# SutirthaChakraborty/RTFS-Net

Hardware: AMD Instinct MI355X
Metric: mixtures/sec forward (2 s@16 kHz, 2-spk) RTFS-Net-4 (higher is better)
Workload: dtype f32 (f16x3 split-precision MFMA products, f32 accumulate; every tensor in HBM is f32)

## Files before the change

### include/rtfs_amd.h

```cpp
#ifndef RTFS_AMD_H
#define RTFS_AMD_H
#include <stddef.h>
#ifdef __cplusplus
extern "C" {
#endif

enum rtfs_pack_kind {
    RTFS_PACK_ENCODER = 0,
    RTFS_PACK_AUDIO_BN = 1,
    RTFS_PACK_BLOCK = 2,
    RTFS_PACK_DUALPATH = 3,
    RTFS_PACK_ATTENTION = 4,
    RTFS_PACK_TFAR = 5,
    RTFS_PACK_CAF = 6,
    RTFS_PACK_S3 = 7,
    RTFS_PACK_DECODER = 8,
    RTFS_PACK_BLOCK_LSTM = 9,
    RTFS_PACK_DUALPATH_LSTM = 10
};

const char* rtfs_version(void);
size_t rtfs_pack_floats(int kind);
int rtfs_num_frames(int L);

// ... 20 lines not shown
int rtfs_tf_attention_f32(const float* x, const float* pack, float* out, int B, int T, void* ws, size_t ws_bytes,
                          void* stream);

size_t rtfs_tfar_workspace_bytes(int B, int H, int W, int Hg, int Wg);
int rtfs_tfar_f32(const float* local, const float* global, const float* pack, float* out, int B, int H, int W, int Hg,
                  int Wg, void* ws, size_t ws_bytes, void* stream);

size_t rtfs_caf_workspace_bytes(int B, int Tv);
int rtfs_caf_f32(const float* audio, const float* video, const float* pack, float* out, int B, int T, int F, int Tv,
                 void* ws, size_t ws_bytes, void* stream);

size_t rtfs_vp_pack_floats(void);
int rtfs_vp_block_f32(const float* video, const float* pack, float* out, int B, int Tv, void* stream);

int rtfs_s3_mask_f32(const float* refined, const float* a0, const float* pack, float* out, int B, int T, int F,
                     void* stream);

size_t rtfs_istft_decoder_workspace_bytes(int B, int T);
int rtfs_istft_decoder_f32(const float* x, const float* pack, float* wav, int B, int T, int L, void* ws, size_t ws_bytes,
                           void* stream);

size_t rtfs_separator_workspace_bytes(int B, int L, int Tv);
int rtfs_set_batch_split(int n);
size_t rtfs_separator_workspace_bytes_ex(int B, int L, int Tv, int split);
int rtfs_separator_forward_ex_f32(const float* wav, const float* video_vp, const float* pack_enc, const float* pack_bn,
                                  const float* pack_block, const float* pack_caf, const float* pack_s3,
                                  const float* pack_dec, float* out, int B, int L, int Tv, int repeats, void* ws,
                                  size_t ws_bytes, void* stream, void* video_ready, int rnn_kind, int split);
int rtfs_separator_forward_f32(const float* wav, const float* video_vp, const float* pack_enc, const float* pack_bn,
                               const float* pack_block, const float* pack_caf, const float* pack_s3,
                               const float* pack_dec, float* out, int B, int L, int Tv, int repeats, void* ws,
                               size_t ws_bytes, void* stream, void* video_ready, int rnn_kind );

size_t rtfs_separator_speakers_workspace_bytes(int B, int K, int L, int Tv, int split);
int rtfs_separator_speakers_f32(const float* wav, const float* video_vp, const float* pack_enc, const float* pack_bn,
                                const float* pack_block, const float* pack_caf, const float* pack_s3, const float* pack_dec,
                                float* out, int B, int K, int L, int Tv, int repeats, void* ws, size_t ws_bytes, void* stream,
                                void* video_ready, int rnn_kind, int split);

size_t rtfs_separator_targets_workspace_bytes(const int* counts, int B, int L, int Tv, int split);
int rtfs_separator_targets_f32(const float* wav, const float* video_vp, const int* counts, const int* mix_of, const float* pack_enc,
                               const float* pack_bn, const float* pack_block, const float* pack_caf, const float* pack_s3,
                               const float* pack_dec, float* out, int B, int N, int L, int Tv, int repeats, void* ws, size_t ws_bytes,
                               void* stream, void* video_ready, int rnn_kind, int split);

size_t rtfs_sru_workspace_bytes(int L, int N);
// ... 269 lines not shown
```

### rtfs-net_amd/_lib.py

```python
from __future__ import annotations

import ctypes as C
import os
import threading

import torch

_HERE = os.path.dirname(os.path.abspath(__file__))
LIB_PATH = os.path.join(_HERE, "librtfs_amd.so")

PACK_ENCODER, PACK_AUDIO_BN, PACK_BLOCK, PACK_DUALPATH, PACK_ATTENTION, PACK_TFAR, PACK_CAF, PACK_S3, PACK_DECODER, PACK_BLOCK_LSTM, PACK_DUALPATH_LSTM = range(11)

_ERR = {-1: "bad shape", -2: "workspace too small", -3: "kernel launch failure", -4: "bad argument"}

_p, _i, _z = C.c_void_p, C.c_int, C.c_size_t
SIGNATURES = {
    "rtfs_version": (C.c_char_p, []),
    "rtfs_pack_floats": (_z, [_i]),
    "rtfs_num_frames": (_i, [_i]),
    "rtfs_stft_encoder_workspace_bytes": (_z, [_i, _i]),
    "rtfs_stft_encoder_f32": (_i, [_p, _p, _p, _p, _i, _i, _p, _z, _p]),
    "rtfs_audio_bottleneck_workspace_bytes": (_z, [_i]),
    "rtfs_audio_bottleneck_f32": (_i, [_p, _p, _p, _p, _i, _i, _i, _p, _z, _p]),
    "rtfs_block_workspace_bytes": (_z, [_i, _i, _i]),
    "rtfs_block_f32": (_i, [_p, _p, _p, _p, _i, _i, _i, _p, _z, _p, _i]),
    "rtfs_dualpath_workspace_bytes": (_z, [_i, _i, _i]),
    "rtfs_dualpath_sru_f32": (_i, [_p, _p, _p, _i, _i, _i, _i, _p, _z, _p]),
    "rtfs_dualpath_lstm_f32": (_i, [_p, _p, _p, _i, _i, _i, _i, _p, _z, _p]),
    "rtfs_tf_attention_workspace_bytes": (_z, [_i, _i]),
    "rtfs_tf_attention_f32": (_i, [_p, _p, _p, _i, _i, _p, _z, _p]),
    "rtfs_tfar_workspace_bytes": (_z, [_i, _i, _i, _i, _i]),
    "rtfs_tfar_f32": (_i, [_p, _p, _p, _p, _i, _i, _i, _i, _i, _p, _z, _p]),
    "rtfs_caf_workspace_bytes": (_z, [_i, _i]),
    "rtfs_caf_f32": (_i, [_p, _p, _p, _p, _i, _i, _i, _i, _p, _z, _p]),
    "rtfs_vp_pack_floats": (_z, []),
    "rtfs_vp_block_f32": (_i, [_p, _p, _p, _i, _i, _p]),
    "rtfs_s3_mask_f32": (_i, [_p, _p, _p, _p, _i, _i, _i, _p]),
    "rtfs_istft_decoder_workspace_bytes": (_z, [_i, _i]),
    "rtfs_istft_decoder_f32": (_i, [_p, _p, _p, _i, _i, _i, _p, _z, _p]),
    "rtfs_separator_workspace_bytes": (_z, [_i, _i, _i]),
    "rtfs_set_batch_split": (_i, [_i]),
    "rtfs_debug_launch_count": (C.c_ulonglong, []),
    "rtfs_separator_workspace_bytes_ex": (_z, [_i, _i, _i, _i]),
    "rtfs_separator_forward_ex_f32": (_i, [_p] * 9 + [_i, _i, _i, _i, _p, _z, _p, _p, _i, _i]),
    "rtfs_separator_forward_f32": (_i, [_p] * 9 + [_i, _i, _i, _i, _p, _z, _p, _p, _i]),
    "rtfs_separator_speakers_workspace_bytes": (_z, [_i, _i, _i, _i, _i]),
    "rtfs_separator_speakers_f32": (_i, [_p] * 9 + [_i, _i, _i, _i, _i, _p, _z, _p, _p, _i, _i]),
    "rtfs_separator_targets_workspace_bytes": (_z, [_p, _i, _i, _i, _i]),
    "rtfs_separator_targets_f32": (_i, [_p] * 11 + [_i, _i, _i, _i, _i, _p, _z, _p, _p, _i, _i]),
    "rtfs_sru_workspace_bytes": (_z, [_i, _i]),
    "rtfs_sru_f32": (_i, [_p, _p, _p, _i, _i, _p, _z, _p]),
    "rtfs_sru_train_pack_floats": (_z, []),
    "rtfs_sru_grad_floats": (_z, []),
    "rtfs_sru_saved_floats": (_z, [_i, _i]),
    "rtfs_sru_backward_workspace_bytes": (_z, [_i, _i]),
    "rtfs_sru_forward_train_f32": (_i, [_p, _p, _p, _p, _i, _i, _p]),
    "rtfs_sru_backward_f32": (_i, [_p, _p, _p, _p, _p, _p, _i, _i, _p, _z, _p]),
    **{f"rtfs_dualpath_{infix}{name}": sig for infix in ("", "lstm_", "gru_") for name, sig in (
        ("train_pack_floats", (_z, [])),
        ("grad_floats", (_z, [])),
        ("saved_floats", (_z, [_i, _i, _i, _i])),
        ("train_workspace_bytes", (_z, [_i, _i, _i, _i])),
        ("forward_train_f32", (_i, [_p, _p, _p, _p, _i, _i, _i, _i, _p, _z, _p])),
        ("backward_f32", (_i, [_p, _p, _p, _p, _p, _p, _i, _i, _i, _i, _p, _z, _p])))},
# ... 232 lines not shown
```

### rtfs-net_amd/csrc/api.hip

```cpp
#include "api_common.h"
#include <atomic>
#include <vector>

namespace {

struct Cursor {
    const float* p;
    size_t off = 0;
    explicit Cursor(const float* base) : p(base) {}
    const float* take(size_t n) {
        const float* r = p ? p + off : nullptr;
        off += (n + 63) / 64 * 64;
        return r;
    }
};

struct Fork {
    hipStream_t st = nullptr;
    RtfsSide side{};
    bool open = false;
    int begin(hipStream_t owner, int slot) {
        st = owner;
        CHECK(rtfs_side_stream(owner, slot, &side));
        if (hipEventRecord(side.fork, st) != hipSuccess || hipStreamWaitEvent(side.stream, side.fork, 0) != hipSuccess) return RTFS_ERR_LAUNCH;
// ... 309 lines not shown
        a.wt = p.proj_wt;
        a.w16 = p.proj_w16;
        a.bias = p.proj_b;
        a.out = w.x_enc;
        a.gw = p.gw;
        a.gb = p.gb;
        a.slope = p.gslope;
        a.P = P;
        a.cs = w.cs;
        a.tile_ctr = ctr;
        if (caf && !gemm_f32()) {
            a.caf_r = caf->r_out; a.caf_att = caf->att_out;
            a.caf_w_key = caf->w_key; a.caf_bn_key = caf->bn_key; a.caf_w_val = caf->w_val; a.caf_bn_val = caf->bn_val;
            a.caf_T = caf->T; a.caf_F = caf->F; a.caf_Tv = caf->Tv;
        }
        if (gemm_f32()) return launch_pw_gateway_proj(a, B, st);
        const int rc = launch_pws_head4(a, B, st);
        if (rc == RTFS_ERR_ARG) CHECK(launch_pws_gateway_proj(a, B, st));
        else CHECK(rc);
    }
    return RTFS_OK;
}

int block_body(const BlockPack& p, int B, int T, int F, const BlockWs& w, hipStream_t st, bool zero_stats = true) {
    const int Tp = T / 2, Fp = F / 2;
    const int P = T * F, Pg = Tp * Fp;
    const double icF = 1.0 / ((double)CH * P), icG = 1.0 / ((double)CH * Pg);
    typedef BlockWs W;
    constexpr int TH_A = 24, TH_B = 24, TH_C = 12, TH_G = 64, TH_S = 64;
    if (zero_stats && hipMemsetAsync(w.stats, 0, sizeof(double) * W::NSTAT * w.Bfull * 2, st) != hipSuccess) return RTFS_ERR_LAUNCH;
    {
        DwArgs a;
        a.x = w.x_enc;
        a.w[0] = p.ds0_w;
        a.bias[0] = p.ds0_b;
        a.out[0] = w.c0;
        a.stats_out[0] = w.st(W::S_C0, B);
        a.C = CH; a.H = T; a.W = F; a.TH = TH_A; a.cs = w.cs;
        CHECK(launch_dw_s1(a, 1, false, 0, B, st));
    }
    DwArgs s14;
    s14.x = w.c0;
    s14.in_stats = w.st(W::S_C0, B); s14.in_inv_count = icF; s14.in_gamma = p.ds0_g; s14.in_beta = p.ds0_be;
    s14.C = CH; s14.H = T; s14.W = F; s14.TH = 64; s14.Hg = Tp; s14.Wg = Fp; s14.cs = w.cs;
    s14.w[0] = p.fus0.loc_w;
    s14.stats_out[0] = w.st(W::S_L0, B);
    s14.rev = 1;
    DwArgs s3;
    s3.x = w.c0;
    s3.in_stats = w.st(W::S_C0, B); s3.in_inv_count = icF; s3.in_gamma = p.ds0_g; s3.in_beta = p.ds0_be;
    s3.w[0] = p.ds1_w;
    s3.bias[0] = p.ds1_b;
// ... 68 lines not shown
        a.w[0] = p.cat0.emb_w; a.w[1] = p.cat0.gate_w;
        a.out[0] = w.E2; a.out[1] = w.G2;
        a.stats_out[0] = w.st(W::S_E2, B); a.stats_out[1] = w.st(W::S_G2, B);
        a.C = CH; a.H = Tp; a.W = Fp; a.TH = TH_G;
        if (Fp >= 16) {
            CHECK(launch_dw_s1(a, 2, false, 0, B, st));
        } else {
            GCombineArgs g;
            g.l = w.L1; g.gate = w.G1; g.emb = w.E1;
            g.l_stats = a.loc_stats; g.gate_stats = a.gate_stats; g.emb_stats = a.emb_stats;
            g.l_gamma = a.loc_gamma; g.l_beta = a.loc_beta; g.gate_gamma = a.gate_gamma; g.gate_beta = a.gate_beta; g.emb_gamma = a.emb_gamma; g.emb_beta = a.emb_beta;
            g.inv_count = icG;
            g.out = w.xf1;
            g.C = CH; g.HW = Pg;
            CHECK(launch_g_combine(g, B, st));
            a.x = w.xf1; a.gate = nullptr; a.emb = nullptr; a.in_combine = 0;
            CHECK(launch_dw_s1(a, 2, false, 0, B, st));
        }
    }
    DwArgs d0in;
    d0in.x = w.c0;
    d0in.in_stats = w.st(W::S_C0, B); d0in.in_inv_count = icF; d0in.in_gamma = p.ds0_g; d0in.in_beta = p.ds0_be;
    d0in.C = CH; d0in.H = T; d0in.W = F; d0in.TH = 64; d0in.Hg = Tp; d0in.Wg = Fp; d0in.cs = w.cs;
    {
        DwArgs a = d0in;
        a.w[0] = p.fus0.loc_w;
        a.loc_stats = w.st(W::S_L0, B); a.loc_inv_count = icF; a.loc_gamma = p.fus0.loc_g; a.loc_beta = p.fus0.loc_b;
        a.gate = w.G0; a.gate_stats = w.st(W::S_G0, B); a.gate_gamma = p.fus0.gate_g; a.gate_beta = p.fus0.gate_b;
        a.emb = w.E0; a.emb_stats = w.st(W::S_E0, B); a.emb_gamma = p.fus0.emb_g; a.emb_beta = p.fus0.emb_b;
        a.g_inv_count = icG;
        a.out[0] = w.xf0;
        a.TH = TH_B;
        CHECK(launch_dw_s1(a, 1, true, 2, B, st));
    }
    DwArgs xin;
    xin.x = w.xf0;
    xin.C = CH; xin.H = T; xin.W = F; xin.TH = 64; xin.Hg = Tp; xin.Wg = Fp; xin.cs = w.cs;
    {
        DwArgs a = xin;
        a.w[0] = p.cat0.loc_w;
        a.stats_out[0] = w.st(W::S_L2, B);
        a.rev = 1;
        a.TH = TH_S;
        CHECK(launch_dw_s1(a, 1, false, 1, B, st));
    }
    {
        DwArgs a = xin;
        a.w[0] = p.cat0.loc_w;
        a.loc_stats = w.st(W::S_L2, B); a.loc_inv_count = icF; a.loc_gamma = p.cat0.loc_g; a.loc_beta = p.cat0.loc_b;
        a.gate = w.G2; a.gate_stats = w.st(W::S_G2, B); a.gate_gamma = p.cat0.gate_g; a.gate_beta = p.cat0.gate_b;
        a.emb = w.E2; a.emb_stats = w.st(W::S_E2, B); a.emb_gamma = p.cat0.emb_g; a.emb_beta = p.cat0.emb_b;
        a.g_inv_count = icG;
        a.addend = w.c0; a.add_stats = w.st(W::S_C0, B); a.add_inv_count = icF; a.add_gamma = p.ds0_g; a.add_beta = p.ds0_be;
        a.out[0] = w.expanded;
        a.rev = 1;
        a.TH = TH_B;
        CHECK(launch_dw_s1(a, 1, false, 2, B, st));
    }
    return RTFS_OK;
}

int block_tail(const BlockPack& p, float* out, int B, int T, int F, BlockWs& w, hipStream_t st, unsigned* ctr = nullptr) {
    const int P = T * F;
    {
        PwArgs a;
        a.x = w.expanded;
        a.wt = p.res_wt;
        a.w16 = p.res_w16;
        a.bias = p.res_b;
        a.aux = w.residual;
        a.out = out;
        a.P = P;
        a.cs = w.cs;
        a.tile_ctr = ctr;
        CHECK(gemm_f32() ? launch_pw_residual(a, B, st) : launch_pws_residual(a, B, st));
    }
    return RTFS_OK;
}

int block_forward(const BlockPack& p, const float* x, const float* x_res, float* out, int B, int T, int F, BlockWs& w, hipStream_t st,
                  const CafArgs* caf = nullptr) {
// ... 481 lines not shown
                CHECK(block_tail(pk, cur, B, T, NF, w.blk, st, f.tile_ctr));
            }
        }
    }
    if (!gemm_f32()) {
        PwArgs a;
        a.x = cur; a.bias = ps.bias; a.aux = w.a0; a.out = w.z; a.slope = ps.slope; a.P = P; a.cs = cs; a.w16 = ps.w16; a.w16b = pd.w16p; a.cout_live = 18;
        a.tile_ctr = nctr < 64 ? w.ctr + nctr++ : nullptr;
        a.stats = w.st0; a.inv_count = 1.0 / ((double)CA * P);
        CHECK(launch_pwr_s3_taps(a, B, st));
        return launch_dec_istft(w.z, out, B, T, NF, L, (size_t)cs, (size_t)18 * cs, st);
    }
    CHECK(s3_mask(ps, cur, w.a0, nxt, B, P, st));
    return decoder(pd, nxt, out, w.z, B, T, L, st);
}
}

static std::atomic<int> g_split{0};
int rtfs_set_batch_split(int n) {
    if (n < 0 || n > 8) return RTFS_ERR_ARG;
    g_split.store(n);
    return RTFS_OK;
}
static int separator_parts(int B, int split = 0) {
    static const int env = getenv("RTFS_SPLIT") ? atoi(getenv("RTFS_SPLIT")) : 0;
    int n = split > 0 ? split : g_split.load();
    if (n <= 0) n = env > 0 ? env : 1;
    while (n > 1 && B / n < 8) --n;
    return n;
}

size_t rtfs_separator_workspace_bytes(int B, int L, int Tv) { return rtfs_separator_workspace_bytes_ex(B, L, Tv, 0); }

size_t rtfs_separator_workspace_bytes_ex(int B, int L, int Tv, int split) {
    if (split < 0 || split > 8) return 0;
    Arena ar(nullptr, 0);
    const int T = rtfs_num_frames(L), np = separator_parts(B, split);
    for (int i = 0; i < np; ++i) SepWs w(ar, (B * (i + 1)) / np - (B * i) / np, T, Tv, pitch(T * NF));
    return ar.off + 256;
}

int rtfs_separator_forward_f32(const float* wav, const float* video_vp, const float* pack_enc, const float* pack_bn, const float* pack_block,
                               const float* pack_caf, const float* pack_s3, const float* pack_dec, float* out, int B, int L, int Tv,
                               int repeats, void* ws, size_t ws_bytes, void* stream, void* video_ready, int rnn_kind) {
    return rtfs_separator_forward_ex_f32(wav, video_vp, pack_enc, pack_bn, pack_block, pack_caf, pack_s3, pack_dec, out, B, L, Tv, repeats, ws, ws_bytes,
                                         stream, video_ready, rnn_kind, 0);
// ... 150 lines not shown
    a.in_stats = (const double*)p[1]; a.in_gamma = (const float*)p[2]; a.in_beta = (const float*)p[3];
    for (int k = 0; k < 4; ++k) {
        a.w[k] = (const float*)p[4 + k];
        a.bias[k] = (present >> k) & 1 ? (const float*)p[8 + k] : nullptr;
        a.out[k] = (float*)p[12 + k];
        a.stats_out[k] = (double*)p[16 + k];
    }
    a.loc_stats = (const double*)p[20]; a.loc_gamma = (const float*)p[21]; a.loc_beta = (const float*)p[22];
    a.gate = (const float*)p[23]; a.gate_stats = (const double*)p[24]; a.gate_gamma = (const float*)p[25]; a.gate_beta = (const float*)p[26];
    a.emb = (const float*)p[27]; a.emb_stats = (const double*)p[28]; a.emb_gamma = (const float*)p[29]; a.emb_beta = (const float*)p[30];
    if ((present >> 4) & 1) {
        a.addend = (const float*)p[31]; a.add_stats = (const double*)p[32]; a.add_gamma = (const float*)p[33]; a.add_beta = (const float*)p[34];
    }
    a.C = n[1]; a.H = n[2]; a.W = n[3]; a.Hg = n[4]; a.Wg = n[5]; a.TH = n[6]; a.cs = n[7]; a.rev = n[8]; a.in_combine = n[12];
    a.in_inv_count = d[0]; a.loc_inv_count = d[1]; a.g_inv_count = d[2]; a.add_inv_count = d[3];
    return a;
}
}

int rtfs_debug_dw_f32(int op, void* const* ptrs, int n_ptrs, const int* ints, int n_ints, const double* dbls, int n_dbls, int* route,
                      int route_cap, void* stream) {
    RTFS_RETURN_IF(!ptrs || !ints || !dbls || !route || route_cap < 1 + 8 * 4, RTFS_ERR_ARG);
    route[0] = 0;
    const int jobs = op == 1 || op == 2 ? 2 : 1;
    int rc;
    if (op >= 0 && op <= 3) {
        RTFS_RETURN_IF(n_ptrs < jobs * DW_DBG_PTRS || n_ints < jobs * DW_DBG_INTS || n_dbls < jobs * DW_DBG_DBLS, RTFS_ERR_ARG);
        const int B = ints[0];
        RTFS_RETURN_IF(B < 1 || ints[1] < 1 || ints[2] < 1 || ints[3] < 1, RTFS_ERR_ARG);
        const DwArgs a = dw_debug_args(ptrs, ints, dbls);
        if (op == 0) {
            rc = launch_dw_s1(a, ints[9], ints[10] != 0, ints[11], B, S(stream));
        } else if (op == 3) {
            rc = launch_dw_s2_pool(a, B, S(stream));
        } else {
            const DwArgs b = dw_debug_args(ptrs + DW_DBG_PTRS, ints + DW_DBG_INTS, dbls + DW_DBG_DBLS);
            rc = op == 1 ? launch_dw_g3(a, b, B, S(stream)) : launch_dw_s2_stats(a, b, B, S(stream));
        }
    } else if (op == 4) {
        RTFS_RETURN_IF(n_ptrs < 6 || n_ints < 3 || n_dbls < 1 || ints[0] < 1 || ints[1] < 1 || ints[2] < 1, RTFS_ERR_ARG);
        rc = launch_g_form((const float*)ptrs[0], (const float*)ptrs[1], (const double*)ptrs[2], dbls[0], (const float*)ptrs[3],
                           (const float*)ptrs[4], (float*)ptrs[5], ints[0], ints[1], ints[2], S(stream));
    } else if (op == 5) {
        RTFS_RETURN_IF(n_ptrs < 13 || n_ints < 3 || n_dbls < 1 || ints[0] < 1 || ints[1] < 1 || ints[2] < 1, RTFS_ERR_ARG);
        GCombineArgs g;
        g.l = (const float*)ptrs[0]; g.gate = (const float*)ptrs[1]; g.emb = (const float*)ptrs[2];
        g.l_stats = (const double*)ptrs[3]; g.gate_stats = (const double*)ptrs[4]; g.emb_stats = (const double*)ptrs[5];
        g.l_gamma = (const float*)ptrs[6]; g.l_beta = (const float*)ptrs[7]; g.gate_gamma = (const float*)ptrs[8];
        g.gate_beta = (const float*)ptrs[9]; g.emb_gamma = (const float*)ptrs[10]; g.emb_beta = (const float*)ptrs[11];
        g.out = (float*)ptrs[12];
        g.inv_count = dbls[0];
        g.C = ints[1]; g.HW = ints[2];
        rc = launch_g_combine(g, ints[0], S(stream));
    } else {
        return RTFS_ERR_ARG;
    }
    const DwRoute& r = dw_route_last();
    route[0] = r.n;
    for (int i = 0; i < r.n; ++i) {
        const DwRouteJob& j = r.job[i];
        const int v[8] = {j.family, j.nconv, j.in_affine, j.mode, j.var, j.TH, j.gx, j.gy};
// ... 230 lines not shown
```

### rtfs-net_amd/csrc/k_dw.hip

```cpp
#include "common.h"
#include "kernels.h"

template <int NCONV, bool IN_AFFINE, int MODE>
__device__ __forceinline__ void dw_s1_body(const DwArgs& a, const float* __restrict__ X, const float* __restrict__ GATE,
                                           const float* __restrict__ EMB, const float* __restrict__ ADD, float* __restrict__ O0,
                                           float* __restrict__ O1, float* __restrict__ O2, float* __restrict__ O3) {
    __shared__ double red[8];
    const int H = a.H, W = a.W, C = a.C;
    const int b = blockIdx.z;
    const int g = blockIdx.x * 256 + threadIdx.x;
    const bool live = g < C * W;
    const int c = live ? g / W : 0, f = live ? g - c * W : 0;
    const int r0 = blockIdx.y * a.TH, r1 = min(r0 + a.TH, H);
    const size_t plane = ((size_t)b * C + c) * (size_t)a.cs;
    const float* __restrict__ xp = X + plane;
    float isc = 1.f, ish = 0.f;
    if (IN_AFFINE) gln_fold(a.in_stats + 2 * b, a.in_inv_count, a.in_gamma[c], a.in_beta[c], isc, ish);
    float wgt[NCONV][16], bia[NCONV];
#pragma unroll
    for (int n = 0; n < NCONV; ++n) {
#pragma unroll
        for (int j = 0; j < 16; ++j) wgt[n][j] = a.w[n][c * 16 + j];
        bia[n] = a.bias[n] ? a.bias[n][c] : 0.f;
    }
// ... 452 lines not shown
    if (MODE != 2) {
#pragma unroll
        for (int n = 0; n < NCONV; ++n) {
            block_stats_atomic(s2[n].x + s2[n].y, ss2[n].x + ss2[n].y, red, a.stats_out[n] + 2 * b);
            __syncthreads();
        }
    }
}

template <int NCONV, bool IN_AFFINE, int MODE, int VAR = 0>
__global__ __launch_bounds__(256, NCONV == 1 && MODE != 2 ? 4 : 2) void dw1p_kernel(DwArgs a) {
    dw1p_body<NCONV, IN_AFFINE, MODE, VAR>(a, a.x, a.gate, a.emb, a.addend, a.out[0], a.out[1], a.out[2], a.out[3]);
}

template <int V>
__global__ __launch_bounds__(256, 2) void dw_g3_kernel(DwArgs a0, DwArgs a1, DwArgs a2) {
    int id = blockIdx.x;
    if (DW_XCD) id = (id & 7) * (int)(gridDim.x >> 3) + (id >> 3);
    if (id < a1.blk0) dw1p_body<2, false, 0, V>(a0, a0.x, a0.gate, a0.emb, a0.addend, a0.out[0], a0.out[1], a0.out[2], a0.out[3]);
    else if (id < a2.blk0) dw1p_body<2, false, 0, V>(a1, a1.x, a1.gate, a1.emb, a1.addend, a1.out[0], a1.out[1], a1.out[2], a1.out[3]);
    else dw1p_body<1, true, 0, V>(a2, a2.x, a2.gate, a2.emb, a2.addend, a2.out[0], a2.out[1], a2.out[2], a2.out[3]);
}

__device__ __forceinline__ void dw_s2_pool_body(const DwArgs& a, const float* __restrict__ X, float* __restrict__ O0, float* __restrict__ O1) {
    __shared__ double red[8];
    const int H = a.H, W = a.W, C = a.C, Ho = a.Hg, Wo = a.Wg;
    const int b = blockIdx.z;
    const int g = blockIdx.x * 256 + threadIdx.x;
    const bool live = g < C * Wo;
    const int c = live ? g / Wo : 0, j = live ? g - c * Wo : 0;
    const int i0 = blockIdx.y * a.TH, i1 = min(i0 + a.TH, Ho);
    const size_t plane = ((size_t)b * C + c) * (size_t)a.cs;
    const float* __restrict__ xp = X + plane;
    float isc, ish;
    gln_fold(a.in_stats + 2 * b, a.in_inv_count, a.in_gamma[c], a.in_beta[c], isc, ish);
    float wgt[16];
#pragma unroll
    for (int k = 0; k < 16; ++k) wgt[k] = a.w[0][c * 16 + k];
    const float bia = a.bias[0][c];
    const int fs = (int)(((long long)j * W) / Wo), fe = (int)(((long long)(j + 1) * W + Wo - 1) / Wo);
    bool fok[4], fpool[4];
    int fcl[4];
#pragma unroll
    for (int d = 0; d < 4; ++d) {
        const int f = 2 * j - 1 + d;
        fok[d] = live && f >= 0 && f < W;
// ... 403 lines not shown
            if (nconv == 2) return a.in_combine ? launch_dw1p_t<2, false, 0, 4>(a, B, st) : launch_dw1p_t<2, false, 0>(a, B, st);
            if (nconv == 4) {
                DwArgs b = a;
                for (int i = 0; i < 2; ++i) {
                    b.w[i] = a.w[2 + i]; b.bias[i] = a.bias[2 + i]; b.out[i] = a.out[2 + i]; b.stats_out[i] = a.stats_out[2 + i];
                }
                const int rc = launch_dw1p_t<2, false, 0>(a, B, st);
                return rc ? rc : launch_dw1p_t<2, false, 0>(b, B, st);
            }
        }
    }
    if (mode == 0 && nconv == 1 && !in_affine) return launch_dw_s1_t<1, false, 0>(a, B, st);
    if (mode == 0 && nconv == 1 && in_affine) return launch_dw_s1_t<1, true, 0>(a, B, st);
    if (mode == 0 && nconv == 2 && !in_affine) return launch_dw_s1_t<2, false, 0>(a, B, st);
    if (mode == 0 && nconv == 4 && !in_affine) return launch_dw_s1_t<4, false, 0>(a, B, st);
    if (mode == 0 && nconv == 3 && !in_affine) return launch_dw_s1_t<3, false, 0>(a, B, st);
    if (mode == 1 && nconv == 1 && in_affine) return launch_dw_s1_t<1, true, 1>(a, B, st);
    if (mode == 1 && nconv == 1 && !in_affine) return launch_dw_s1_t<1, false, 1>(a, B, st);
    if (mode == 2 && nconv == 1 && in_affine) return launch_dw_s1_t<1, true, 2>(a, B, st);
    if (mode == 2 && nconv == 1 && !in_affine) return launch_dw_s1_t<1, false, 2>(a, B, st);
    return RTFS_ERR_ARG;
}

int launch_dw_g3(const DwArgs& conv4, const DwArgs& aff1, int B, hipStream_t st) {
    route_clear();
    DwArgs j[3] = {conv4, conv4, aff1};
    const bool nohalo = 64 % ((conv4.W + 1) / 2) == 0 && conv4.W == aff1.W;
    for (int i = 0; i < 2; ++i) {
        j[1].w[i] = conv4.w[2 + i]; j[1].bias[i] = conv4.bias[2 + i]; j[1].out[i] = conv4.out[2 + i]; j[1].stats_out[i] = conv4.stats_out[2 + i];
    }
    int off = 0;
    for (int i = 0; i < 3; ++i) {
        DwArgs& a = j[i];
        if (a.W < 16 || (a.cs && a.cs < a.H * a.W)) return RTFS_ERR_ARG;
        if (!a.cs) a.cs = a.H * a.W;
        if ((size_t)a.C * a.cs * 4 >= ((size_t)1 << 31)) return RTFS_ERR_ARG;
        a.rev = 0;
        a.gx = cdiv(cdiv(a.C * ((a.W + 1) / 2), nohalo ? 64 : DW1P_PAIRS), 4);
        a.TH = band_rows(a.TH, a.H, a.gx, 3 * B, 640);
        a.gy = cdiv(a.H, a.TH);
        a.nblk = a.gx * a.gy * B;
        a.blk0 = off;
        off += a.nblk;
    }
    for (int i = 0; i < 3; ++i) route_add(DW_FAM_G3, i < 2 ? 2 : 1, i == 2, 0, nohalo ? 16 : 0, j[i].TH, j[i].gx, j[i].gy);
    if (nohalo) hipLaunchKernelGGL(dw_g3_kernel<16>, dim3((off + 7) / 8 * 8), dim3(256), 0, st, j[0], j[1], j[2]);
// ... 130 lines not shown
```

### rtfs-net_amd/csrc/kernels.h

```cpp
#pragma once
#include <hip/hip_runtime.h>
#include <stddef.h>
#include "common.h"

struct PwArgs {
    const float* x = nullptr;
    const float* x2 = nullptr;
    float* res_out = nullptr;
    const float* wt = nullptr;
    const void* w16 = nullptr;
    const void* w16b = nullptr;
    const float* bias = nullptr;
    const float* aux = nullptr;
    float* out = nullptr;
    const double* stats = nullptr;
    double inv_count = 0;
    const float* gamma = nullptr;
    const float* beta = nullptr;
    const float* gw = nullptr;
    const float* gb = nullptr;
    const float* slope = nullptr;
    int P = 0;
    int cs = 0;
    int cout_live = 0;
// ... 134 lines not shown
    const float* gate_beta = nullptr;
    const float* emb = nullptr;
    const double* emb_stats = nullptr;
    const float* emb_gamma = nullptr;
    const float* emb_beta = nullptr;
    double g_inv_count = 0;
    const float* addend = nullptr;
    const double* add_stats = nullptr;
    double add_inv_count = 0;
    const float* add_gamma = nullptr;
    const float* add_beta = nullptr;
};

struct GCombineArgs {
    const float *l, *gate, *emb;
    const double *l_stats, *gate_stats, *emb_stats;
    const float *l_gamma, *l_beta, *gate_gamma, *gate_beta, *emb_gamma, *emb_beta;
    double inv_count;
    float* out;
    int C, HW;
};

enum DwFamily { DW_FAM_S1 = 1, DW_FAM_1P = 2, DW_FAM_G3 = 3, DW_FAM_S2X = 4, DW_FAM_S2_POOL = 5, DW_FAM_S2_STATS = 6, DW_FAM_G_FORM = 7,
                DW_FAM_G_COMBINE = 8 };
struct DwRouteJob { int family, nconv, in_affine, mode, var, TH, gx, gy; };
struct DwRoute { int n; DwRouteJob job[4]; };
const DwRoute& dw_route_last();

int launch_dw_s1(const DwArgs& a, int nconv, bool in_affine, int mode, int B, hipStream_t st);
int launch_dw_g3(const DwArgs& conv4, const DwArgs& aff1, int B, hipStream_t st);
int launch_dw_s2_pool(const DwArgs& a, int B, hipStream_t st);
int launch_dw_s2_stats(const DwArgs& s2, const DwArgs& stats, int B, hipStream_t st);
int launch_g_form(const float* p0, const float* c1, const double* st1, double inv_count, const float* gamma,
                  const float* beta, float* g, int B, int C, int HW, hipStream_t st);
int launch_g_combine(const GCombineArgs& a, int B, hipStream_t st);
int launch_transpose(const float* x, float* y, int N, int H, int W, hipStream_t st);
int launch_stats(const float* x, double* stats, int B, size_t N, hipStream_t st);
int launch_stats2(const float* x, double* stats, int B, size_t N, double* part, hipStream_t st);

struct DpArgs {
    const float* x = nullptr;
    float* out = nullptr;
    int R = 0, Ls = 0;
    size_t bstride = 0, rstride = 0, cstride = 0;
    const float* ln_gamma = nullptr;
    const float* ln_beta = nullptr;
    const float* W0 = nullptr;
    const float* Wl = nullptr;
    const float* wc = nullptr;
    const float* bias = nullptr;
    const float* Wt = nullptr;
    const float* bt = nullptr;
    const float* whh = nullptr;
};
size_t dualpath_lds_bytes(int Ls);
// ... 308 lines not shown
```

Baseline: 3338.

## Fuse fusion, concat-stats and concat-output depthwise stages into a two-pass recompute kernel

Adds a two-pass depthwise kernel for the W=129 case that recomputes the gated fusion output xf0 on the fly in a per-wave LDS ring, instead of writing xf0 to HBM and reading it back twice. Pass 0 computes only the concat-branch statistics; pass 1 recomputes xf0, applies the second conv, gate, embedding and residual, then stages output rows through an LDS ring for coalesced stores. It is enabled when the activation footprint exceeds 256 MB, or when forced through a new API setter. Otherwise the original three launches remain. The trade-off is extra arithmetic from recomputing xf0 twice, against saving its HBM traffic at large batch.

```diff
diff --git a/include/rtfs_amd.h b/include/rtfs_amd.h
--- a/include/rtfs_amd.h
+++ b/include/rtfs_amd.h
@@ -66,6 +66,7 @@
 
 size_t rtfs_separator_workspace_bytes(int B, int L, int Tv);
 int rtfs_set_batch_split(int n);
+int rtfs_set_dw_two_pass(int mode);
 size_t rtfs_separator_workspace_bytes_ex(int B, int L, int Tv, int split);
 int rtfs_separator_forward_ex_f32(const float* wav, const float* video_vp, const float* pack_enc, const float* pack_bn,
                                   const float* pack_block, const float* pack_caf, const float* pack_s3,
diff --git a/rtfs-net_amd/_lib.py b/rtfs-net_amd/_lib.py
--- a/rtfs-net_amd/_lib.py
+++ b/rtfs-net_amd/_lib.py
@@ -40,6 +40,7 @@
     "rtfs_istft_decoder_f32": (_i, [_p, _p, _p, _i, _i, _i, _p, _z, _p]),
     "rtfs_separator_workspace_bytes": (_z, [_i, _i, _i]),
     "rtfs_set_batch_split": (_i, [_i]),
+    "rtfs_set_dw_two_pass": (_i, [_i]),
     "rtfs_debug_launch_count": (C.c_ulonglong, []),
     "rtfs_separator_workspace_bytes_ex": (_z, [_i, _i, _i, _i]),
     "rtfs_separator_forward_ex_f32": (_i, [_p] * 9 + [_i, _i, _i, _i, _p, _z, _p, _p, _i, _i]),
diff --git a/rtfs-net_amd/csrc/api.hip b/rtfs-net_amd/csrc/api.hip
--- a/rtfs-net_amd/csrc/api.hip
+++ b/rtfs-net_amd/csrc/api.hip
@@ -355,12 +355,21 @@
     return RTFS_OK;
 }
 
+static std::atomic<int> g_dw_two_pass{0};
+#ifndef RTFS_DW2P_TH_A
+#define RTFS_DW2P_TH_A 64
+#endif
+#ifndef RTFS_DW2P_TH_B
+#define RTFS_DW2P_TH_B 64
+#endif
+constexpr size_t DW_TWO_PASS_BYTES = 256u * 1000u * 1000u;
 int block_body(const BlockPack& p, int B, int T, int F, const BlockWs& w, hipStream_t st, bool zero_stats = true) {
     const int Tp = T / 2, Fp = F / 2;
     const int P = T * F, Pg = Tp * Fp;
     const double icF = 1.0 / ((double)CH * P), icG = 1.0 / ((double)CH * Pg);
     typedef BlockWs W;
     constexpr int TH_A = 24, TH_B = 24, TH_C = 12, TH_G = 64, TH_S = 64;
+    constexpr int TH_2A = RTFS_DW2P_TH_A, TH_2B = RTFS_DW2P_TH_B;
     if (zero_stats && hipMemsetAsync(w.stats, 0, sizeof(double) * W::NSTAT * w.Bfull * 2, st) != hipSuccess) return RTFS_ERR_LAUNCH;
     {
         DwArgs a;
@@ -475,41 +484,48 @@
     d0in.x = w.c0;
     d0in.in_stats = w.st(W::S_C0, B); d0in.in_inv_count = icF; d0in.in_gamma = p.ds0_g; d0in.in_beta = p.ds0_be;
     d0in.C = CH; d0in.H = T; d0in.W = F; d0in.TH = 64; d0in.Hg = Tp; d0in.Wg = Fp; d0in.cs = w.cs;
-    {
-        DwArgs a = d0in;
-        a.w[0] = p.fus0.loc_w;
-        a.loc_stats = w.st(W::S_L0, B); a.loc_inv_count = icF; a.loc_gamma = p.fus0.loc_g; a.loc_beta = p.fus0.loc_b;
-        a.gate = w.G0; a.gate_stats = w.st(W::S_G0, B); a.gate_gamma = p.fus0.gate_g; a.gate_beta = p.fus0.gate_b;
-        a.emb = w.E0; a.emb_stats = w.st(W::S_E0, B); a.emb_gamma = p.fus0.emb_g; a.emb_beta = p.fus0.emb_b;
-        a.g_inv_count = icG;
-        a.out[0] = w.xf0;
-        a.TH = TH_B;
-        CHECK(launch_dw_s1(a, 1, true, 2, B, st));
-    }
+    DwArgs f0 = d0in;
+    f0.w[0] = p.fus0.loc_w;
+    f0.loc_stats = w.st(W::S_L0, B); f0.loc_inv_count = icF; f0.loc_gamma = p.fus0.loc_g; f0.loc_beta = p.fus0.loc_b;
+    f0.gate = w.G0; f0.gate_stats = w.st(W::S_G0, B); f0.gate_gamma = p.fus0.gate_g; f0.gate_beta = p.fus0.gate_b;
+    f0.emb = w.E0; f0.emb_stats = w.st(W::S_E0, B); f0.emb_gamma = p.fus0.emb_g; f0.emb_beta = p.fus0.emb_b;
+    f0.g_inv_count = icG;
     DwArgs xin;
     xin.x = w.xf0;
     xin.C = CH; xin.H = T; xin.W = F; xin.TH = 64; xin.Hg = Tp; xin.Wg = Fp; xin.cs = w.cs;
-    {
-        DwArgs a = xin;
-        a.w[0] = p.cat0.loc_w;
-        a.stats_out[0] = w.st(W::S_L2, B);
-        a.rev = 1;
-        a.TH = TH_S;
-        CHECK(launch_dw_s1(a, 1, false, 1, B, st));
-    }
-    {
-        DwArgs a = xin;
-        a.w[0] = p.cat0.loc_w;
-        a.loc_stats = w.st(W::S_L2, B); a.loc_inv_count = icF; a.loc_gamma = p.cat0.loc_g; a.loc_beta = p.cat0.loc_b;
-        a.gate = w.G2; a.gate_stats = w.st(W::S_G2, B); a.gate_gamma = p.cat0.gate_g; a.gate_beta = p.cat0.gate_b;
-        a.emb = w.E2; a.emb_stats = w.st(W::S_E2, B); a.emb_gamma = p.cat0.emb_g; a.emb_beta = p.cat0.emb_b;
-        a.g_inv_count = icG;
-        a.addend = w.c0; a.add_stats = w.st(W::S_C0, B); a.add_inv_count = icF; a.add_gamma = p.ds0_g; a.add_beta = p.ds0_be;
-        a.out[0] = w.expanded;
-        a.rev = 1;
-        a.TH = TH_B;
-        CHECK(launch_dw_s1(a, 1, false, 2, B, st));
-    }
+    DwArgs s16 = xin;
+    s16.w[0] = p.cat0.loc_w;
+    s16.stats_out[0] = w.st(W::S_L2, B);
+    DwArgs s17 = xin;
+    s17.w[0] = p.cat0.loc_w;
+    s17.loc_stats = w.st(W::S_L2, B); s17.loc_inv_count = icF; s17.loc_gamma = p.cat0.loc_g; s17.loc_beta = p.cat0.loc_b;
+    s17.gate = w.G2; s17.gate_stats = w.st(W::S_G2, B); s17.gate_gamma = p.cat0.gate_g; s17.gate_beta = p.cat0.gate_b;
+    s17.emb = w.E2; s17.emb_stats = w.st(W::S_E2, B); s17.emb_gamma = p.cat0.emb_g; s17.emb_beta = p.cat0.emb_b;
+    s17.g_inv_count = icG;
+    s17.addend = w.c0; s17.add_stats = w.st(W::S_C0, B); s17.add_inv_count = icF; s17.add_gamma = p.ds0_g; s17.add_beta = p.ds0_be;
+    s17.out[0] = w.expanded;
+    const int two_pass = g_dw_two_pass.load();
+    if (two_pass == 2 || (two_pass == 0 && (size_t)B * CH * w.cs * sizeof(float) > DW_TWO_PASS_BYTES)) {
+        s16.TH = TH_2A;
+        s16.rev = 0;
+        const int rc = launch_dw_two_pass(f0, s16, 0, B, st);
+        if (rc == RTFS_OK) {
+            s17.TH = TH_2B;
+            s17.rev = 1;
+            const int rc2 = launch_dw_two_pass(f0, s17, 1, B, st);
+            return rc2 == RTFS_ERR_ARG ? RTFS_ERR_SHAPE : rc2;
+        }
+        if (rc != RTFS_ERR_ARG) return rc;
+    }
+    f0.out[0] = w.xf0;
+    f0.TH = TH_B;
+    CHECK(launch_dw_s1(f0, 1, true, 2, B, st));
+    s16.rev = 1;
+    s16.TH = TH_S;
+    CHECK(launch_dw_s1(s16, 1, false, 1, B, st));
+    s17.rev = 1;
+    s17.TH = TH_B;
+    CHECK(launch_dw_s1(s17, 1, false, 2, B, st));
     return RTFS_OK;
 }
 
@@ -1037,6 +1053,11 @@
     g_split.store(n);
     return RTFS_OK;
 }
+int rtfs_set_dw_two_pass(int mode) {
+    if (mode < 0 || mode > 2) return RTFS_ERR_ARG;
+    g_dw_two_pass.store(mode);
+    return RTFS_OK;
+}
 static int separator_parts(int B, int split = 0) {
     static const int env = getenv("RTFS_SPLIT") ? atoi(getenv("RTFS_SPLIT")) : 0;
     int n = split > 0 ? split : g_split.load();
@@ -1233,7 +1254,7 @@
                       int route_cap, void* stream) {
     RTFS_RETURN_IF(!ptrs || !ints || !dbls || !route || route_cap < 1 + 8 * 4, RTFS_ERR_ARG);
     route[0] = 0;
-    const int jobs = op == 1 || op == 2 ? 2 : 1;
+    const int jobs = op == 1 || op == 2 || op == 6 || op == 7 ? 2 : 1;
     int rc;
     if (op >= 0 && op <= 3) {
         RTFS_RETURN_IF(n_ptrs < jobs * DW_DBG_PTRS || n_ints < jobs * DW_DBG_INTS || n_dbls < jobs * DW_DBG_DBLS, RTFS_ERR_ARG);
@@ -1248,6 +1269,12 @@
             const DwArgs b = dw_debug_args(ptrs + DW_DBG_PTRS, ints + DW_DBG_INTS, dbls + DW_DBG_DBLS);
             rc = op == 1 ? launch_dw_g3(a, b, B, S(stream)) : launch_dw_s2_stats(a, b, B, S(stream));
         }
+    } else if (op == 6 || op == 7) {
+        RTFS_RETURN_IF(n_ptrs < 2 * DW_DBG_PTRS || n_ints < 2 * DW_DBG_INTS || n_dbls < 2 * DW_DBG_DBLS, RTFS_ERR_ARG);
+        RTFS_RETURN_IF(ints[0] < 1 || ints[1] < 1 || ints[2] < 1 || ints[3] < 1, RTFS_ERR_ARG);
+        const DwArgs a = dw_debug_args(ptrs, ints, dbls);
+        const DwArgs b = dw_debug_args(ptrs + DW_DBG_PTRS, ints + DW_DBG_INTS, dbls + DW_DBG_DBLS);
+        rc = launch_dw_two_pass(a, b, op - 6, ints[0], S(stream));
     } else if (op == 4) {
         RTFS_RETURN_IF(n_ptrs < 6 || n_ints < 3 || n_dbls < 1 || ints[0] < 1 || ints[1] < 1 || ints[2] < 1, RTFS_ERR_ARG);
         rc = launch_g_form((const float*)ptrs[0], (const float*)ptrs[1], (const double*)ptrs[2], dbls[0], (const float*)ptrs[3],
diff --git a/rtfs-net_amd/csrc/k_dw.hip b/rtfs-net_amd/csrc/k_dw.hip
--- a/rtfs-net_amd/csrc/k_dw.hip
+++ b/rtfs-net_amd/csrc/k_dw.hip
@@ -498,6 +498,313 @@
     else dw1p_body<1, true, 0, V>(a2, a2.x, a2.gate, a2.emb, a2.addend, a2.out[0], a2.out[1], a2.out[2], a2.out[3]);
 }
 
+template <int PASS>
+__device__ __forceinline__ void dw2p_body(const DwArgs& a, const DwArgs& c2) {
+    __shared__ double red[8];
+    constexpr int W = 129, XR = 132, RING = 2048;
+    constexpr unsigned W4 = W * 4u;
+    __shared__ __attribute__((aligned(16))) float xring_all[4][4 * XR];
+    __shared__ __attribute__((aligned(16))) unsigned char oring_all[PASS ? 4 : 1][PASS ? RING : 16];
+    const int H = a.H, C = a.C;
+    const DwBlk blk = dw_block(a);
+    if (!blk.ok) return;
+    const int b = blk.z;
+    const int lane = threadIdx.x & 63, wave = threadIdx.x >> 6;
+    const int c = blk.x * 4 + wave;
+    const int r0 = blk.y * a.TH, r1 = min(r0 + a.TH, H);
+    const unsigned pa = (unsigned)c * (unsigned)a.cs * 4u;
+    const unsigned vld = pa + 8u * (unsigned)lane;
+    const unsigned vex = pa + 4u * (unsigned)(W - 1);
+    const size_t sample = (size_t)b * C * (size_t)a.cs;
+    const BufRsrc xs = buf_rsrc(a.x + sample);
+    const BufRsrc os = buf_rsrc(PASS ? c2.out[0] + sample : a.x);
+    const size_t gsample = (size_t)b * C * a.Hg * a.Wg;
+    const BufRsrc gs = buf_rsrc(a.gate + gsample), es = buf_rsrc(a.emb + gsample);
+    const BufRsrc gs2 = buf_rsrc(PASS ? c2.gate + gsample : a.gate), es2 = buf_rsrc(PASS ? c2.emb + gsample : a.emb);
+    const unsigned gpa = (unsigned)c * (unsigned)(a.Hg * a.Wg) * 4u;
+    const unsigned sc0 = min((unsigned)(2 * lane) * (unsigned)a.Wg / (unsigned)W, (unsigned)a.Wg - 1u);
+    const unsigned sc1 = min((unsigned)(2 * lane + 1) * (unsigned)a.Wg / (unsigned)W, (unsigned)a.Wg - 1u);
+    const bool gnext = sc1 != sc0;
+    const unsigned fga = gpa + 4u * (lane == 0 ? min((unsigned)(W - 1) * (unsigned)a.Wg / (unsigned)W, (unsigned)a.Wg - 1u) : sc0);
+    const bool border = r0 < 2 || r1 + 4 > H;
+    const int sA = max(r0 - 1, 0);
+    int qa = (int)(((long long)sA * a.Hg) / H), ra = (int)(((long long)sA * a.Hg) % H);
+    int qb = (int)(((long long)r0 * a.Hg) / H), rb = (int)(((long long)r0 * a.Hg) % H);
+    struct Raw { f32x2 pr; float xe, g0, m0, g2, m2; int tg0, tg2; };
+    auto load_raw = [&](int L) {
+        const int tc = L < 0 ? 0 : (L < H ? L : H - 1);
+        Raw r;
+        r.pr = buf_ld2(xs, vld, (unsigned)tc * W4);
+        r.xe = buf_ld1(xs, vex, (unsigned)tc * W4);
+        {
+            const int tg = qa < a.Hg - 1 ? qa : a.Hg - 1;
+            ra += L - 2 >= sA ? a.Hg : 0;
+            const bool wrap = ra >= H;
+            ra -= wrap ? H : 0;
+            qa += wrap ? 1 : 0;
+            const unsigned grow = (unsigned)tg * (unsigned)a.Wg * 4u;
+            r.g0 = buf_ld1(gs, fga, grow);
+            r.m0 = buf_ld1(es, fga, grow);
+            r.tg0 = tg;
+        }
+        r.g2 = r.m2 = 0.f;
+        r.tg2 = 0;
+        if (PASS) {
+            const int tg = qb < a.Hg - 1 ? qb : a.Hg - 1;
+            rb += L - 4 >= r0 ? a.Hg : 0;
+            const bool wrap = rb >= H;
+            rb -= wrap ? H : 0;
+            qb += wrap ? 1 : 0;
+            const unsigned grow = (unsigned)tg * (unsigned)a.Wg * 4u;
+            r.g2 = buf_ld1(gs2, fga, grow);
+            r.m2 = buf_ld1(es2, fga, grow);
+            r.tg2 = tg;
+        }
+        return r;
+    };
+    struct Row { f32x2 p[4]; float xe; };
+    auto complete = [&](int L, const Raw& r) {
+        const float v1 = r.pr.x, v2 = r.pr.y;
+        const float v0 = from_prev_lane(v2), v4 = from_next_lane(v2);
+        float v3 = from_next_lane(v1);
+        v3 = lane == 63 ? r.xe : v3;
+        Row w;
+        w.xe = r.xe;
+        w.p[0] = f32x2{v0, v1};
+        w.p[1] = f32x2{v1, v2};
+        w.p[2] = f32x2{v2, v3};
+        w.p[3] = f32x2{v3, v4};
+        if (border && (L < 0 || L >= H)) {
+#pragma unroll
+            for (int j = 0; j < 4; ++j) w.p[j] = f32x2{0.f, 0.f};
+            w.xe = 0.f;
+        }
+        return w;
+    };
+    constexpr int RQ = 4;
+    constexpr int QD = 2;
+    Raw st0 = load_raw(r0 - 2), st1 = load_raw(r0 - 1), st2 = load_raw(r0);
+    Raw q[QD];
+#pragma unroll
+    for (int k = 0; k < QD; ++k) q[k] = load_raw(r0 + 1 + k);
+    f32x4 wraw[2][4];
+#pragma unroll
+    for (int i = 0; i < 4; ++i) {
+        wraw[0][i] = *reinterpret_cast<const f32x4*>(a.w[0] + c * 16 + i * 4);
+        wraw[1][i] = *reinterpret_cast<const f32x4*>(c2.w[0] + c * 16 + i * 4);
+    }
+    float isc, ish, lsc, lsh, gsc, gsh, esc, esh;
+    gln_fold(a.in_stats + 2 * b, a.in_inv_count, a.in_gamma[c], a.in_beta[c], isc, ish);
+    gln_fold(a.loc_stats + 2 * b, a.loc_inv_count, a.loc_gamma[c], a.loc_beta[c], lsc, lsh);
+    gln_fold(a.gate_stats + 2 * b, a.g_inv_count, a.gate_gamma[c], a.gate_beta[c], gsc, gsh);
+    gln_fold(a.emb_stats + 2 * b, a.g_inv_count, a.emb_gamma[c], a.emb_beta[c], esc, esh);
+    gsc = first_lane_f(gsc); gsh = first_lane_f(gsh);
+    esc = first_lane_f(esc); esh = first_lane_f(esh);
+    float l2sc = 1.f, l2sh = 0.f, g2sc = 1.f, g2sh = 0.f, e2sc = 1.f, e2sh = 0.f, asc = 1.f, ash = 0.f;
+    if (PASS) {
+        gln_fold(c2.loc_stats + 2 * b, c2.loc_inv_count, c2.loc_gamma[c], c2.loc_beta[c], l2sc, l2sh);
+        gln_fold(c2.gate_stats + 2 * b, c2.g_inv_count, c2.gate_gamma[c], c2.gate_beta[c], g2sc, g2sh);
+        gln_fold(c2.emb_stats + 2 * b, c2.g_inv_count, c2.emb_gamma[c], c2.emb_beta[c], e2sc, e2sh);
+        gln_fold(c2.add_stats + 2 * b, c2.add_inv_count, c2.add_gamma[c], c2.add_beta[c], asc, ash);
+        g2sc = first_lane_f(g2sc); g2sh = first_lane_f(g2sh);
+        e2sc = first_lane_f(e2sc); e2sh = first_lane_f(e2sh);
+        asc = first_lane_f(asc); ash = first_lane_f(ash);
+    }
+    f32x2 wp[16];
+#pragma unroll
+    for (int j = 0; j < 4; ++j) {
+        const int xa = 2 * lane - 1 + j, xb = 2 * lane + j;
+        const bool okA = xa >= 0 && xa < W, okB = xb < W;
+#pragma unroll
+        for (int i = 0; i < 4; ++i) {
+            wp[i * 4 + j] = f32x2{okA ? wraw[0][i][j] : 0.f, okB ? wraw[0][i][j] : 0.f};
+            asm volatile("" : "+v"(wp[i * 4 + j]));
+        }
+    }
+    auto rowsum = [&](int i) { return (wp[i * 4] + wp[i * 4 + 1]) + (wp[i * 4 + 2] + wp[i * 4 + 3]); };
+    const f32x2 wv_full = (rowsum(0) + rowsum(1)) + (rowsum(2) + rowsum(3));
+    const float bv0 = a.bias[0] ? a.bias[0][c] : 0.f, bv1 = c2.bias[0] ? c2.bias[0][c] : 0.f;
+    const f32x2 bias0 = f32x2{bv0, bv0}, bias1 = f32x2{bv1, bv1};
+    const float bias0_e = first_lane_f(bv0), bias1_e = first_lane_f(bv1);
+    float we0[4], we1[4], rse[4], w2s[4][4];
+#pragma unroll
+    for (int i = 0; i < 4; ++i) {
+        we0[i] = first_lane_f(wraw[0][i][0]);
+        we1[i] = first_lane_f(wraw[0][i][1]);
+        rse[i] = we0[i] + we1[i];
+#pragma unroll
+        for (int j = 0; j < 4; ++j) w2s[i][j] = first_lane_f(wraw[1][i][j]);
+    }
+    const float wve_full = (rse[0] + rse[1]) + (rse[2] + rse[3]);
+    float* const xring = xring_all[wave];
+    if (lane < 4) {
+        xring[lane * XR] = 0.f;
+        xring[lane * XR + W + 1] = 0.f;
+        xring[lane * XR + W + 2] = 0.f;
+    }
+    unsigned char* const oring = oring_all[PASS ? wave : 0];
+    const unsigned s0 = (unsigned)r0 * W4, s1 = (unsigned)r1 * W4;
+    unsigned chunk = s0 >> 9;
+    auto flush = [&](unsigned cidx) {
+        const unsigned cb = cidx << 9, b0 = cb + 8u * (unsigned)lane;
+        const f32x2 v = *reinterpret_cast<const f32x2*>(oring + (cb & (RING - 1)) + 8u * (unsigned)lane);
+        if (cb >= s0 && cb + 512u <= s1) {
+            buf_st2(os, pa + 8u * (unsigned)lane, cb, v);
+        } else {
+            if (b0 >= s0 && b0 + 4u <= s1) buf_st1(os, pa + 8u * (unsigned)lane, cb, v.x);
+            if (b0 + 4u >= s0 && b0 + 8u <= s1) buf_st1(os, pa + 8u * (unsigned)lane + 4u, cb, v.y);
+        }
+    };
+    auto stage = [&](int t, f32x2 y, float ye) {
+        const unsigned pos = (unsigned)t * W4 + 8u * (unsigned)lane;
+        *reinterpret_cast<float*>(oring + (pos & (RING - 1))) = y.x;
+        *reinterpret_cast<float*>(oring + ((pos + 4u) & (RING - 1))) = y.y;
+        if (lane == 63) *reinterpret_cast<float*>(oring + ((pos + 8u) & (RING - 1))) = ye;
+        const unsigned end = (unsigned)(t + 1) * W4;
+        while (((chunk + 1u) << 9) <= end) {
+            flush(chunk);
+            ++chunk;
+        }
+    };
+    auto lane63_f = [](float v) { return __int_as_float(__builtin_amdgcn_readlane(__float_as_int(v), 63)); };
+    auto gate_emb = [&](float gv, float mv, float sc_g, float sh_g, float sc_e, float sh_e, f32x2& gate, f32x2& emb) {
+        float g0 = gv, m0 = mv;
+        float gn = from_next_lane(gv), mn = from_next_lane(mv);
+        const float ge = lane0_f(gv), me = lane0_f(mv);
+        g0 = lane == 0 ? gn : g0;
+        m0 = lane == 0 ? mn : m0;
+        gn = lane == 63 ? ge : gn;
+        mn = lane == 63 ? me : mn;
+        const float g1 = gnext ? gn : g0, m1 = gnext ? mn : m0;
+        gate = f32x2{sigmoidf_(fmaf(g0, sc_g, sh_g)), sigmoidf_(fmaf(g1, sc_g, sh_g))};
+        emb = f32x2{fmaf(m0, sc_e, sh_e), fmaf(m1, sc_e, sh_e)};
+    };
+    f32x2 gateA = {0.f, 0.f}, embA = {0.f, 0.f}, gateB = {0.f, 0.f}, embB = {0.f, 0.f};
+    int rowA = -1, rowB = -1;
+    constexpr bool KEEP_GATES = PASS == 1;
+    auto xf0_row = [&](int u, int slot, const Row& w0, const Row& w1, const Row& w2, const Row& w3, const Raw& e) {
+        f32x2 accA = w0.p[0] * wp[0], accB = w2.p[0] * wp[8];
+#pragma unroll
+        for (int j = 1; j < 4; ++j) {
+            accA = w0.p[j] * wp[j] + accA;
+            accB = w2.p[j] * wp[8 + j] + accB;
+        }
+#pragma unroll
+        for (int j = 0; j < 4; ++j) {
+            accA = w1.p[j] * wp[4 + j] + accA;
+            accB = w3.p[j] * wp[12 + j] + accB;
+        }
+        f32x2 acc = accA + accB;
+        float ea = fmaf(w0.xe, we1[0], w0.p[1].y * we0[0]), eb = fmaf(w2.xe, we1[2], w2.p[1].y * we0[2]);
+        ea = fmaf(w1.xe, we1[1], fmaf(w1.p[1].y, we0[1], ea));
+        eb = fmaf(w3.xe, we1[3], fmaf(w3.p[1].y, we0[3], eb));
+        float acce = ea + eb;
+        f32x2 wv = wv_full;
+        float wve = wve_full;
+        if (border) {
+            if (u - 1 < 0) { wv -= rowsum(0); wve -= rse[0]; }
+            if (u + 1 >= H) { wv -= rowsum(2); wve -= rse[2]; }
+            if (u + 2 >= H) { wv -= rowsum(3); wve -= rse[3]; }
+        }
+        acc = acc * isc + wv * ish;
+        acce = fmaf(acce, isc, wve * ish);
+        acc += bias0;
+        acce += bias0_e;
+        if (!KEEP_GATES || e.tg0 != rowA) {
+            gate_emb(e.g0, e.m0, gsc, gsh, esc, esh, gateA, embA);
+            rowA = e.tg0;
+        }
+        f32x2 y = (acc * lsc + lsh) * gateA + embA;
+        float ye = fmaf(fmaf(acce, lsc, lsh), lane63_f(gateA.y), lane63_f(embA.y));
+        if (border && (u < 0 || u >= H)) {
+            y = f32x2{0.f, 0.f};
+            ye = 0.f;
+        }
+        float* const rp = xring + slot * XR + 1 + 2 * lane;
+        rp[0] = y.x;
+        rp[1] = y.y;
+        if (lane == 63) rp[2] = ye;
+    };
+    f32x2 s2 = {0.f, 0.f}, ss2 = {0.f, 0.f};
+    auto out_row = [&](int t, int k0, const Raw& e, f32x2 dpr, float dxe) {
+        float v[4][5];
+#pragma unroll
+        for (int i = 0; i < 4; ++i) {
+            const float* const rp = xring + ((k0 + i) & 3) * XR + 2 * lane;
+            const f32x2 lo = *reinterpret_cast<const f32x2*>(rp), hi = *reinterpret_cast<const f32x2*>(rp + 2);
+            v[i][0] = lo.x; v[i][1] = lo.y; v[i][2] = hi.x; v[i][3] = hi.y; v[i][4] = rp[4];
+        }
+        float a0 = v[0][0] * w2s[0][0], a1 = v[0][1] * w2s[0][0], b0 = v[2][0] * w2s[2][0], b1 = v[2][1] * w2s[2][0];
+#pragma unroll
+        for (int j = 1; j < 4; ++j) {
+            a0 = fmaf(v[0][j], w2s[0][j], a0); a1 = fmaf(v[0][j + 1], w2s[0][j], a1);
+            b0 = fmaf(v[2][j], w2s[2][j], b0); b1 = fmaf(v[2][j + 1], w2s[2][j], b1);
+        }
+#pragma unroll
+        for (int j = 0; j < 4; ++j) {
+            a0 = fmaf(v[1][j], w2s[1][j], a0); a1 = fmaf(v[1][j + 1], w2s[1][j], a1);
+            b0 = fmaf(v[3][j], w2s[3][j], b0); b1 = fmaf(v[3][j + 1], w2s[3][j], b1);
+        }
+        f32x2 acc = f32x2{a0 + b0, a1 + b1};
+        float ea = fmaf(v[0][3], w2s[0][1], v[0][2] * w2s[0][0]), eb = fmaf(v[2][3], w2s[2][1], v[2][2] * w2s[2][0]);
+        ea = fmaf(v[1][3], w2s[1][1], fmaf(v[1][2], w2s[1][0], ea));
+        eb = fmaf(v[3][3], w2s[3][1], fmaf(v[3][2], w2s[3][0], eb));
+        float acce = ea + eb;
+        acc += bias1;
+        acce += bias1_e;
+        if (!PASS) {
+            s2 += acc;
+            ss2 = acc * acc + ss2;
+            const float em = lane == 63 ? acce : 0.f;
+            s2.x += em;
+            ss2.x = fmaf(em, em, ss2.x);
+            return;
+        }
+        if (e.tg2 != rowB) {
+            gate_emb(e.g2, e.m2, g2sc, g2sh, e2sc, e2sh, gateB, embB);
+            rowB = e.tg2;
+        }
+        f32x2 y = (acc * l2sc + l2sh) * gateB + embB;
+        y += f32x2{fmaf(dpr.x, asc, ash), fmaf(dpr.y, asc, ash)};
+        float ye = fmaf(fmaf(acce, l2sc, l2sh), lane63_f(gateB.y), lane63_f(embB.y));
+        ye += fmaf(dxe, asc, ash);
+        stage(t, y, ye);
+    };
+    Row win[3];
+    win[0] = complete(r0 - 2, st0);
+    win[1] = complete(r0 - 1, st1);
+    win[2] = complete(r0, st2);
+    f32x2 dpr = {0.f, 0.f};
+    float dxe = 0.f;
+    for (int u = r0 - 1; u < r1 + 2; u += RQ) {
+#pragma unroll
+        for (int k = 0; k < RQ; ++k) {
+            const Raw e = q[k % QD];
+            const Row n = complete(u + k + 2, e);
+            if (u + k < r1 + 2) {
+                xf0_row(u + k, k & 3, win[0], win[1], win[2], n, e);
+                __builtin_amdgcn_wave_barrier();
+                if (u + k - 2 >= r0) out_row(u + k - 2, (k + 1) & 3, e, dpr, dxe);
+                __builtin_amdgcn_wave_barrier();
+            }
+            q[k % QD] = load_raw(u + k + 2 + QD);
+            dpr = win[0].p[1];
+            dxe = win[0].xe;
+            win[0] = win[1];
+            win[1] = win[2];
+            win[2] = n;
+        }
+    }
+    if (PASS) {
+        if ((chunk << 9) < s1) flush(chunk);
+    } else {
+        block_stats_atomic(s2.x + s2.y, ss2.x + ss2.y, red, c2.stats_out[0] + 2 * b);
+    }
+}
+
+template <int PASS>
+__global__ __launch_bounds__(256, PASS ? 3 : 4) void dw2p_kernel(DwArgs a, DwArgs c2) { dw2p_body<PASS>(a, c2); }
+
 __device__ __forceinline__ void dw_s2_pool_body(const DwArgs& a, const float* __restrict__ X, float* __restrict__ O0, float* __restrict__ O1) {
     __shared__ double red[8];
     const int H = a.H, W = a.W, C = a.C, Ho = a.Hg, Wo = a.Wg;
@@ -947,6 +1254,36 @@
     return RTFS_ERR_ARG;
 }
 
+int launch_dw_two_pass(const DwArgs& first, const DwArgs& second, int pass, int B, hipStream_t st) {
+    route_clear();
+    DwArgs a = first;
+    const DwArgs& c = second;
+    if (pass < 0 || pass > 1 || B < 1 || a.W != 129 || a.C < 4 || a.C % 4 != 0 || a.H < 1 || a.Hg < 1 || a.Wg < 1 || c.TH < 1) return RTFS_ERR_ARG;
+    if (c.C != a.C || c.H != a.H || c.W != a.W || c.Hg != a.Hg || c.Wg != a.Wg || c.cs != a.cs) return RTFS_ERR_ARG;
+    if (a.cs && a.cs < a.H * a.W) return RTFS_ERR_ARG;
+    if (!a.cs) a.cs = a.H * a.W;
+    if ((size_t)a.C * a.cs * 4 >= ((size_t)1 << 31)) return RTFS_ERR_ARG;
+    if (!(nearest_is_integer_quotient(a.Hg, a.H) && nearest_is_integer_quotient(a.Wg, a.W))) return RTFS_ERR_ARG;
+    if (!(2 * a.Wg <= a.W && (a.W - 1) * a.Wg / a.W == (a.W - 2) * a.Wg / a.W && 2 * a.Wg / a.W == 0)) return RTFS_ERR_ARG;
+    if (!a.x || !a.in_stats || !a.in_gamma || !a.in_beta || !a.w[0] || !a.loc_stats || !a.loc_gamma || !a.loc_beta || !a.gate || !a.gate_stats ||
+        !a.gate_gamma || !a.gate_beta || !a.emb || !a.emb_stats || !a.emb_gamma || !a.emb_beta || a.addend || !c.w[0])
+        return RTFS_ERR_ARG;
+    if (pass == 0 && !c.stats_out[0]) return RTFS_ERR_ARG;
+    if (pass == 1 && (!c.out[0] || c.addend != a.x || !c.add_stats || !c.add_gamma || !c.add_beta || !c.loc_stats || !c.loc_gamma || !c.loc_beta ||
+                      !c.gate || !c.gate_stats || !c.gate_gamma || !c.gate_beta || !c.emb || !c.emb_stats || !c.emb_gamma || !c.emb_beta))
+        return RTFS_ERR_ARG;
+    a.gx = a.C / 4;
+    a.TH = band_rows(c.TH, a.H, a.gx, B, pass ? 768 : 320);
+    a.gy = cdiv(a.H, a.TH);
+    a.nblk = a.gx * a.gy * B;
+    a.rev = c.rev;
+    a.blk0 = a.job_stride = a.job_off = 0;
+    route_add(DW_FAM_2P, 2, 1, pass ? 2 : 1, pass ? 11 : 10, a.TH, a.gx, a.gy);
+    if (pass) hipLaunchKernelGGL(dw2p_kernel<1>, dim3((a.nblk + 7) / 8 * 8), dim3(256), 0, st, a, c);
+    else hipLaunchKernelGGL(dw2p_kernel<0>, dim3((a.nblk + 7) / 8 * 8), dim3(256), 0, st, a, c);
+    return rtfs_launch_status();
+}
+
 int launch_dw_g3(const DwArgs& conv4, const DwArgs& aff1, int B, hipStream_t st) {
     route_clear();
     DwArgs j[3] = {conv4, conv4, aff1};
diff --git a/rtfs-net_amd/csrc/kernels.h b/rtfs-net_amd/csrc/kernels.h
--- a/rtfs-net_amd/csrc/kernels.h
+++ b/rtfs-net_amd/csrc/kernels.h
@@ -180,7 +180,7 @@
 };
 
 enum DwFamily { DW_FAM_S1 = 1, DW_FAM_1P = 2, DW_FAM_G3 = 3, DW_FAM_S2X = 4, DW_FAM_S2_POOL = 5, DW_FAM_S2_STATS = 6, DW_FAM_G_FORM = 7,
-                DW_FAM_G_COMBINE = 8 };
+                DW_FAM_G_COMBINE = 8, DW_FAM_2P = 9 };
 struct DwRouteJob { int family, nconv, in_affine, mode, var, TH, gx, gy; };
 struct DwRoute { int n; DwRouteJob job[4]; };
 const DwRoute& dw_route_last();
@@ -189,6 +189,7 @@
 int launch_dw_g3(const DwArgs& conv4, const DwArgs& aff1, int B, hipStream_t st);
 int launch_dw_s2_pool(const DwArgs& a, int B, hipStream_t st);
 int launch_dw_s2_stats(const DwArgs& s2, const DwArgs& stats, int B, hipStream_t st);
+int launch_dw_two_pass(const DwArgs& first, const DwArgs& second, int pass, int B, hipStream_t st);
 int launch_g_form(const float* p0, const float* c1, const double* st1, double inv_count, const float* gamma,
                   const float* beta, float* g, int B, int C, int HW, hipStream_t st);
 int launch_g_combine(const GCombineArgs& a, int B, hipStream_t st);
```

New measurement: 3398 (median of 6 runs). 1.8% higher.
